# lovelyqian/Embodied-One-Shot-Video-Recognition

Measured on AMD Instinct MI355X. Metric: clips/sec/GPU (224², 8-seg) + 5-way-1-shot episode acc vs reference, higher is better.
Workload: dtype f32

## Files before the change

embodied-one-shot-video-recognition_amd/csrc/common.h:

```cpp
#pragma once

#include <hip/hip_runtime.h>

#include "eosv.h"

#include <cstdint>
#include <string>

namespace eosv {

#ifndef EOSV_BF16_RFIRST
#define EOSV_BF16_RFIRST 1
#endif

template <int N>
__device__ __forceinline__ void vm_wait() {
  static_assert(N >= 0 && N < 64, "vmcnt range");
  __builtin_amdgcn_s_waitcnt((N & 15) | ((N >> 4) << 14) | (7 << 4) | (15 << 8));
  asm volatile("" ::: "memory");
}

template <class V>
__device__ __forceinline__ void store_b128_guarded(V v, __amdgpu_buffer_rsrc_t r, int voff, int soff) {
#ifdef EOSV_STORE_GUARD_SB
  __builtin_amdgcn_sched_barrier(0);
  __builtin_amdgcn_raw_buffer_store_b128(v, r, voff, soff, 0);
  __builtin_amdgcn_sched_barrier(0);
  asm volatile("s_nop 0");
  __builtin_amdgcn_sched_barrier(0);
#elif defined(EOSV_STORE_GUARD_OFF)
  __builtin_amdgcn_raw_buffer_store_b128(v, r, voff, soff, 0);
#else
  __builtin_amdgcn_raw_buffer_store_b128(v, r, voff, soff, 0);
  asm volatile("s_nop 0" ::"v"(v));
#endif
}

namespace epi {
typedef float f32x2 __attribute__((ext_vector_type(2)));
typedef float f32x4 __attribute__((ext_vector_type(4)));
typedef __bf16 bf16x2 __attribute__((ext_vector_type(2)));
typedef short s16x2 __attribute__((ext_vector_type(2)));
__device__ __forceinline__ unsigned relu_bf2(f32x2 v) {
  const s16x2 h = __builtin_bit_cast(s16x2, __builtin_convertvector(v, bf16x2));
  return __builtin_bit_cast(unsigned, __builtin_elementwise_max(h, (s16x2){0, 0}));
}
__device__ __forceinline__ f32x2 bf2_f(unsigned u) {
  return (f32x2){__uint_as_float(u << 16), __uint_as_float(u & 0xffff0000u)};
}
__device__ __forceinline__ f32x2 pair_of(const f32x4& A, const f32x4& B, int k) {
  const f32x4 X = k >> 1 ? B : A;
  return k & 1 ? X.hi : X.lo;
}
}

void set_error(const std::string& msg);

#ifdef EOSV_PROFILING
int env_switch(const char* name, int dflt);
#define EOSV_ABL(a) ((a).abl)
#else
constexpr int env_switch(const char*, int dflt) { return dflt; }
#define EOSV_ABL(a) 0
#endif

#define EOSV_HIP_CHECK(expr)                                                               \
  do {                                                                                     \
    hipError_t _e = (expr);                                                                \
    if (_e != hipSuccess) {                                                                \
      ::eosv::set_error(std::string(#expr) + ": " + hipGetErrorString(_e));               \
      return EOSV_ERR_HIP;                                                                 \
    }                                                                                      \
  } while (0)

#define EOSV_LAUNCH_CHECK()                                                                \
  do {                                                                                     \
    hipError_t _e = hipGetLastError();                                                     \
    if (_e != hipSuccess) {                                                                \
      ::eosv::set_error(std::string("kernel launch: ") + hipGetErrorString(_e));          \
      return EOSV_ERR_HIP;                                                                 \
    }                                                                                      \
  } while (0)

struct LaunchInfo {
  long long blocks;
  long long slots;
};
int device_cu_count();
int kernel_occupancy(const void* kernel, int threads, size_t dyn_lds = 0);
inline int record_launch(LaunchInfo* info, long long blocks, long long per_cu) {
  info->blocks = blocks;
  info->slots = per_cu * device_cu_count();
  return EOSV_OK;
}

struct ConvArgs {
  const void* x;
  const void* w;
  const float* bias;
  const void* res;
  void* y;
  int N, H, W, Cin;
  int Ho, Wo, Cout;
  int KH, KW, KWp, stride, pad;
  int K;
  int relu;
  const void* zero;
  int abl;
  int xcd;
  int kcm;
  const void* x2;
  int H2, W2, Cin2, stride2, K1;
  int split;
  int xs, x2s;
  LaunchInfo* plan;
  float* kws;
  long long kws_bytes;
};
int conv_f32_ksplit_slices(const ConvArgs& a);

__host__ __device__ inline int split_chan(int c, int cin3) {
  const int c2 = 2 * (cin3 / 3);
  return c >= c2 ? c - c2 : c;
}
inline void conv_pixel_strides(ConvArgs& a) {
  if (!a.xs) a.xs = a.split ? 2 * (a.Cin / 3) : a.Cin;
  if (!a.x2s) a.x2s = a.split ? 2 * (a.Cin2 / 3) : a.Cin2;
}

__device__ __forceinline__ int xcd_tile(int b, int nb, int on) {
  if (!on) return b;
  const int q = nb >> 3, r = nb & 7, x = b & 7, i = b >> 3;
  return x * q + (x < r ? x : r) + i;
}

int launch_conv_f32(const ConvArgs& a, hipStream_t s);
int launch_conv_bf16(const ConvArgs& a, hipStream_t s);
bool conv_bf16_ts_ok(const ConvArgs& a);
int launch_conv_bf16_ts(const ConvArgs& a, hipStream_t s);
bool stem_pool_bf16_ok(int H, int W, bool direct);
int launch_stem_pool_bf16(const void* pack, int B, int H, int W, const void* w, const float* bias, void* y,
                          hipStream_t s, const float* frames = nullptr, LaunchInfo* info = nullptr);
bool stem_pool_x3_ok(int H, int W);
int launch_stem_pool_x3(const float* frames, int B, int H, int W, const void* w, const float* bias, void* y,
                        hipStream_t s, LaunchInfo* info = nullptr);
bool stem_pool_f32_ok(int H, int W);
bool stem_pool_f32_direct_ok(int H, int W);
int launch_stem_pool_f32(const void* pack, int B, int H, int W, const void* w, const float* bias, void* y,
                         hipStream_t s, bool split = false,
                         LaunchInfo* info = nullptr,
                         const float* frames = nullptr);
bool conv_rows_bf16_ok(const ConvArgs& a);
int launch_conv_rows_bf16(const ConvArgs& a, hipStream_t s);
bool conv_rowsr_bf16_ok(const ConvArgs& a);
int launch_conv_rowsr_bf16(const ConvArgs& a, hipStream_t s);
bool conv_s2rows_bf16_ok(const ConvArgs& a);
int launch_conv_s2rows_bf16(const ConvArgs& a, hipStream_t s);

struct Pair1x1Args {
  const void* x;
  const void* x2;
  const void* res;
  const void* w3;
  const float* b3;
  const void* w1;
  const float* b1;
  void* y;
  void* z;
  long long M;
  int c1, cds;
  LaunchInfo* plan;
  int cmid, cexp;
  int Ho, Wo, H2, W2;
  int abl;
  long long cap_elems;
};
bool pair1x1_bf16_ok(int cmid, int cexp, int c1, int cds, long long M);
int launch_pair1x1_bf16(const Pair1x1Args& a, hipStream_t s);
int launch_pair1x1r_bf16(const Pair1x1Args& a, hipStream_t s);
int pairw_tile(int cmid, int c1, int cds);
bool pairw_bf16_ok(int cmid, int cexp, int c1, int cds, long long M, long long cap_elems);
int launch_pairw_bf16(const Pair1x1Args& a, hipStream_t s);
struct BneckArgs {
  const void* x;
  const void* w1; const float* b1;
  const void* w2; const float* b2;
  const void* w3; const float* b3;
  const void* wn; const float* bn;
  void* y;
  void* z;
  int N, H, W, cin;
  LaunchInfo* plan;
  const void* res;
  int abl;
};
bool bneck_bf16_ok(int cin, int W, int H, int next);
int launch_bneck_bf16(const BneckArgs& a, hipStream_t s);
bool bneck_tail_bf16_ok(int W, int H);
int launch_bneck_tail_bf16(const BneckArgs& a, hipStream_t s);
bool bblock_bf16_ok(int W, int H);
int launch_bblock_bf16(const BneckArgs& a, hipStream_t s);
bool conv_rows_f32_ok(const ConvArgs& a);
int launch_conv_rows_f32(const ConvArgs& a, hipStream_t s);
bool conv_rows_x3_ok(const ConvArgs& a);
int launch_conv_rows_x3(const ConvArgs& a, hipStream_t s);

struct WinoDiv {
  unsigned m;
  int s;
};
inline WinoDiv wino_div(unsigned d) {
  int l = 0;
  while ((1ull << l) < d) ++l;
  return {(unsigned)((1ull << (31 + l)) / d + 1), 31 + l};
}
__host__ __device__ inline int wino_fdiv(int t, WinoDiv f) {
  return (int)(((unsigned long long)(unsigned)t * f.m) >> f.s);
}
struct WinoArgs {
  const float* x;
  const float* u;
  const float* bias;
  const float* res;
  float* y;
  int N, H, W, C;
  int relu;
  int xcd;
  int cbmajor;
  LaunchInfo* plan;
  int max_wg;
  WinoDiv dtt, dtw, dncb, dnmt;
};
inline size_t wino_u_index(int o, int i, int pos, int cin) {
  return ((((size_t)(o / 64) * (cin / 8) + i / 8) * 16 + pos) * 8 + i % 8) * 64 + o % 64;
}
bool conv_wino_f32_ok(int C);
int launch_conv_wino_f32(const WinoArgs& a, hipStream_t s);

__host__ __device__ inline int stem_row_pixels(int W, int pad) { return (W + 2 * pad + 1) & ~1; }
inline size_t stem_input_elems(int B, int H, int W, int pad) {
  return (size_t)B * (H + 2 * pad) * stem_row_pixels(W, pad) * 3 + 64;
}
int launch_pack_rgb_pad(const float* x, int B, int H, int W, int pad, void* y, int bf16, hipStream_t s);
int launch_maxpool3x3s2(const void* x, int B, int H, int W, int C, void* y, int Ho, int Wo,
                        int bf16, hipStream_t s);
int launch_avgpool(const void* x, int B, int HW, int C, float* y, int bf16, hipStream_t s);
int launch_act_to_f32(const void* x, long long n, int C, int mode, float* y, hipStream_t s);

}
```

embodied-one-shot-video-recognition_amd/csrc/eosv_api.hip:

```cpp
#include <hip/hip_bf16.h>

#include <cmath>
#include <cstdio>
#include <algorithm>
#include <cstring>
#include <string>
#include <unordered_map>
#include <vector>

#include "common.h"

#ifndef EOSV_F32_KCM_DEF
#define EOSV_F32_KCM_DEF 64
#endif

namespace eosv {

static thread_local std::string g_err;
void set_error(const std::string& msg) { g_err = msg; }

int device_cu_count() {
  static const int n = [] {
    int dev = 0, c = 0;
    if (hipGetDevice(&dev) != hipSuccess || hipDeviceGetAttribute(&c, hipDeviceAttributeMultiprocessorCount, dev) ||
// ... 330 lines not shown
  auto kidx = [&](int i, int y, int x) {
    return c.kcm ? ((size_t)(i / c.kcmc) * c.kh * c.kw + y * c.kw + x) * c.kcmc + i % c.kcmc
                 : ((size_t)y * c.kwp + x) * c.cinp + i;
  };
  for (int o = 0; o < c.cout; ++o)
    for (int i = 0; i < c.cin; ++i)
      for (int y = 0; y < c.kh; ++y)
        for (int x = 0; x < c.kw; ++x) {
          const float v = w[(((size_t)o * c.cin + i) * c.kh + y) * c.kw + x] * alpha[o];
          float* row = wf.data() + (size_t)o * c.K;
          if (!split) {
            row[kidx(i, y, x)] = v;
          } else {
            const float hi = bf_round_host(v);
            row[kidx(i, y, x)] = hi;
            row[kidx(c.cin + i, y, x)] = hi;
            row[kidx(2 * c.cin + i, y, x)] = bf_round_host(v - hi);
          }
        }
  return true;
}

static int upload_conv(eosv_handle* h, Conv& c, const Tensors& t, bool bf16, bool has_bn, Conv* ds = nullptr,
                       bool split = false) {
  std::vector<float> wf, beta, alpha;
  if (!fold_conv(c, t, bf16, has_bn, wf, beta, split, &alpha)) return EOSV_ERR_ARG;
  if (wino_eligible(h, c) && !ds) {
    std::vector<float> u((size_t)16 * c.cout * c.cin);
    const float* w = t.get(c.wname, (int64_t)c.cout * c.cin * 9);
    if (!w || eosv_wino_weights_f32(w, alpha.data(), c.cout, c.cin, u.data())) return EOSV_ERR_ARG;
    int urc;
    if ((urc = upload_bytes(h, (void**)&c.wu, &c.wubytes, u.data(), u.size() * 4))) return urc;
  }
  if (ds) {
    std::vector<float> wd, bd;
    if (!fold_conv(*ds, t, bf16, true, wd, bd, split)) return EOSV_ERR_ARG;
    if (ds->cout != c.cout || ds->kh != 1 || ds->K != c.kds) return set_error("fused downsample shape"), EOSV_ERR_ARG;
    const int Kt = c.K + c.kds;
    std::vector<float> wc((size_t)c.cout * Kt);
    for (int o = 0; o < c.cout; ++o) {
      std::copy(wf.begin() + (size_t)o * c.K, wf.begin() + (size_t)(o + 1) * c.K, wc.begin() + (size_t)o * Kt);
      std::copy(wd.begin() + (size_t)o * c.kds, wd.begin() + (size_t)(o + 1) * c.kds, wc.begin() + (size_t)o * Kt + c.K);
      beta[o] += bd[o];
    }
    wf.swap(wc);
  }
  int rc;
  if (bf16) {
    std::vector<unsigned short> wb(wf.size());
    for (size_t i = 0; i < wf.size(); ++i) wb[i] = f2bf_host(wf[i]);
    if ((rc = upload_bytes(h, &c.w, &c.wbytes, wb.data(), wb.size() * 2))) return rc;
  } else {
    if ((rc = upload_bytes(h, &c.w, &c.wbytes, wf.data(), wf.size() * 4))) return rc;
  }
  size_t bcap = c.b ? (size_t)c.cout * 4 : 0;
  return upload_bytes(h, (void**)&c.b, &bcap, beta.data(), (size_t)c.cout * 4);
}

static hipEvent_t prof_event(eosv_handle* h) {
  if (h->pool_used == h->pool.size()) {
    hipEvent_t e;
    if (hipEventCreate(&e) != hipSuccess) return nullptr;
    h->pool.push_back(e);
  }
  return h->pool[h->pool_used++];
}

static void add_plan_cost(eosv_handle* h, const LaunchInfo& li, double flops) {
  if (li.blocks <= 0 || li.slots <= 0) return;
  const double rounds = (double)((li.blocks + li.slots - 1) / li.slots);
  h->plan_cost += flops * rounds * (double)li.slots / (double)li.blocks;
}

#ifdef EOSV_PROFILING
__global__ __launch_bounds__(256) void lds_poison_kernel() {
  __shared__ unsigned lds[160 * 1024 / 4];
  volatile unsigned* p = lds;
  for (int i = threadIdx.x; i < 160 * 1024 / 4; i += 256) p[i] = 0xffffffffu;
}
static int poison_mode() { return env_switch("EOSV_POISON", 0); }
static void poison_lds(hipStream_t s) {
  if (poison_mode() & 4) (void)hipStreamSynchronize(s);
  if (poison_mode() & 2) hipLaunchKernelGGL(lds_poison_kernel, dim3(4 * device_cu_count()), dim3(256), 0, s);
  if (poison_mode() & 4) (void)hipStreamSynchronize(s);
}
static int poison_bufs(eosv_handle* h, hipStream_t s) {
  if (!(poison_mode() & 1)) return EOSV_OK;
  const size_t elt = act_bytes(h);
  for (void* p : h->buf) EOSV_HIP_CHECK(hipMemsetAsync(p, 0xff, (size_t)h->d.max_frames * h->act_elems * elt, s));
  for (void* p : h->sbuf)
    if (p) EOSV_HIP_CHECK(hipMemsetAsync(p, 0xff, (size_t)h->sub_frames * h->act_elems * elt, s));
  return EOSV_OK;
}
#else
static void poison_lds(hipStream_t) {}
static int poison_bufs(eosv_handle*, hipStream_t) { return EOSV_OK; }
#endif

static int run_conv(eosv_handle* h, const Conv& c, const void* x, int N, int H, int W, const void* res,
                    void* y, bool relu, bool bf16, hipStream_t s, const void* x2 = nullptr, int H2 = 0,
                    int W2 = 0, int stride2 = 1) {
  ConvArgs a{};
  a.x = x;
  a.w = c.w;
  a.bias = c.b;
  a.res = res;
  a.y = y;
  a.N = N;
  a.H = H;
  a.W = W;
  a.Cin = c.cinp;
  a.Ho = conv_out(H, c.kh, c.stride, c.pad);
  a.Wo = conv_out(W, c.kw, c.stride, c.pad);
  a.Cout = c.cout;
  a.KH = c.kh;
  a.KW = c.kw;
  a.KWp = c.kwp;
  a.stride = c.stride;
  a.pad = c.pad;
  a.K = c.K + (x2 ? c.kds : 0);
  a.relu = relu ? 1 : 0;
  if (x2) {
    a.x2 = x2;
    a.H2 = H2;
    a.W2 = W2;
    a.Cin2 = c.kds;
    a.stride2 = stride2;
    a.K1 = c.K;
  }
  a.zero = h->zero;
  static const int xcd = env_switch("EOSV_XCD", 1);
  a.xcd = xcd;
  a.kcm = c.kcm ? (bf16 ? 1 : c.kcmc) : 0;
  a.split = (bf16 && x3(h)) ? 1 : 0;
  a.xs = a.split ? 2 * c.cin : c.cinp;
  a.x2s = x2 ? (a.split ? 2 * (c.kds / 3) : c.kds) : 0;
  const double flops = 2.0 * N * a.Ho * a.Wo * c.cout *
                       ((double)c.kh * c.kw * c.cin + (x2 ? c.kds / (a.split ? 3 : 1) : 0));
  const bool wino = !bf16 && c.wu && !x2;
  WinoArgs wa{};
  if (wino) {
    wa.x = (const float*)x;
    wa.u = c.wu;
    wa.bias = c.b;
    wa.res = (const float*)res;
    wa.y = (float*)y;
    wa.N = N;
    wa.H = H;
    wa.W = W;
    wa.C = c.cin;
    wa.relu = a.relu;
    wa.xcd = xcd;
  }
  if (h->planning) {
    LaunchInfo li{};
    a.plan = wa.plan = &li;
    const int prc = wino ? launch_conv_wino_f32(wa, s) : bf16 ? launch_conv_bf16(a, s) : launch_conv_f32(a, s);
    if (prc == EOSV_OK) add_plan_cost(h, li, flops);
    return prc;
  }
  poison_lds(s);
  hipEvent_t e0 = nullptr, e1 = nullptr;
  if (h->prof) {
    e0 = prof_event(h);
    e1 = prof_event(h);
    if (!e0 || !e1) return set_error("profiling: hipEventCreate failed"), EOSV_ERR_HIP;
    EOSV_HIP_CHECK(hipEventRecord(e0, s));
  }
  const int rc = wino ? launch_conv_wino_f32(wa, s) : bf16 ? launch_conv_bf16(a, s) : launch_conv_f32(a, s);
  if (h->prof && rc == EOSV_OK) {
    EOSV_HIP_CHECK(hipEventRecord(e1, s));
    h->recs.push_back({c.id, e0, e1, flops});
  }
  return rc;
}

static bool pair_enabled() {
  static const bool v = env_switch("EOSV_PAIR", 1) != 0;
  return v;
}

static bool pairw_enabled() {
  static const bool v = env_switch("EOSV_PAIRW", 1) != 0;
  return v;
}

static long long act_buffer_elems(const eosv_handle* h) {
  const long long f = h->sub_frames > 0 ? std::min(h->sub_frames, h->d.max_frames) : h->d.max_frames;
  return f * (long long)h->act_elems;
}

static bool pair_ok(const eosv_handle* h, const Block& b, const Block* nb, long long M) {
  if (!pair_enabled() || !conv_bf(h) || x3(h) || !b.bottleneck || !nb || !nb->bottleneck) return false;
  const Conv &c3 = b.c3, &n1 = nb->c1;
  if (c3.kh != 1 || n1.kh != 1 || n1.stride != 1 || n1.cin != c3.cout) return false;
  if (c3.cin != 64) {
    const bool ds = b.has_ds && b.fuse_ds && b.ds.stride == 2 && b.c2.stride == 2;
    if (!pairw_enabled() || (b.has_ds && !ds)) return false;
    return pairw_bf16_ok(c3.cin, c3.cout, n1.cout, ds ? c3.kds : 0, M, act_buffer_elems(h));
  }
  if (b.c2.stride != 1 || (b.has_ds && !(b.fuse_ds && b.ds.stride == 1))) return false;
  return pair1x1_bf16_ok(c3.cin, c3.cout, n1.cout, b.has_ds ? c3.kds : 0, M);
}

static int run_pair(eosv_handle* h, const Block& b, const Block& nb, const void* x, const void* x2, const void* res,
                    void* y, void* z, long long M, hipStream_t s, int ho = 0, int wo = 0, int hin = 0, int win = 0) {
  Pair1x1Args p{};
  p.x = x;
  p.x2 = x2;
  p.res = res;
  p.w3 = b.c3.w;
  p.b3 = b.c3.b;
  p.w1 = nb.c1.w;
  p.b1 = nb.c1.b;
  p.y = y;
  p.z = z;
  p.M = M;
  p.c1 = nb.c1.cout;
  p.cds = x2 ? b.c3.kds : 0;
  p.cmid = b.c3.cin;
  p.cexp = b.c3.cout;
  p.Ho = ho;
  p.Wo = wo;
  p.H2 = hin;
  p.W2 = win;
  p.cap_elems = act_buffer_elems(h);
  const bool wide = p.cmid != 64;
  const double flops = 2.0 * M * ((double)b.c3.cout * (b.c3.cin + p.cds) + (double)nb.c1.cout * nb.c1.cin);
  if (h->planning) {
    LaunchInfo li{};
    p.plan = &li;
    const int prc = wide ? launch_pairw_bf16(p, s) : launch_pair1x1_bf16(p, s);
    if (prc == EOSV_OK) add_plan_cost(h, li, flops);
    return prc;
  }
  poison_lds(s);
  hipEvent_t e0 = nullptr, e1 = nullptr;
  if (h->prof) {
    e0 = prof_event(h);
    e1 = prof_event(h);
    if (!e0 || !e1) return set_error("profiling: hipEventCreate failed"), EOSV_ERR_HIP;
    EOSV_HIP_CHECK(hipEventRecord(e0, s));
  }
#ifdef EOSV_PROFILING
  static void* scr[3] = {nullptr, nullptr, nullptr};
  static size_t scr_b = 0;
  const bool selfcheck = (poison_mode() & 8) != 0;
  const size_t cap_b = (size_t)p.cap_elems * 2;
  if (selfcheck) {
    if (cap_b > scr_b) {
      for (auto& q : scr) {
        if (q) EOSV_HIP_CHECK(hipFree(q));
        q = nullptr;
        EOSV_HIP_CHECK(hipMalloc(&q, cap_b));
      }
      scr_b = cap_b;
    }
    if (res) EOSV_HIP_CHECK(hipMemcpyAsync(scr[0], res, cap_b, hipMemcpyDeviceToDevice, s));
  }
#endif
  const int rc = wide ? launch_pairw_bf16(p, s) : launch_pair1x1_bf16(p, s);
  if (h->prof && rc == EOSV_OK) {
    EOSV_HIP_CHECK(hipEventRecord(e1, s));
    h->recs.push_back({b.c3.id, e0, e1, flops});
  }
#ifdef EOSV_PROFILING
  if (selfcheck && rc == EOSV_OK) {
    Pair1x1Args q = p;
    if (res) q.res = scr[0];
    q.y = scr[1];
    q.z = scr[2];
    const int rc2 = wide ? launch_pairw_bf16(q, s) : launch_pair1x1_bf16(q, s);
    EOSV_HIP_CHECK(hipStreamSynchronize(s));
    const size_t ny = (size_t)M * p.cexp, nz = (size_t)M * p.c1;
    std::vector<unsigned short> a(ny), c(ny);
    long long dy = 0, dz = 0, fy = -1, fz = -1;
    EOSV_HIP_CHECK(hipMemcpy(a.data(), y, ny * 2, hipMemcpyDeviceToHost));
    EOSV_HIP_CHECK(hipMemcpy(c.data(), scr[1], ny * 2, hipMemcpyDeviceToHost));
    for (size_t i = 0; i < ny; ++i)
      if (a[i] != c[i] && dy++ == 0) fy = (long long)i;
    a.resize(nz);
    c.resize(nz);
    EOSV_HIP_CHECK(hipMemcpy(a.data(), z, nz * 2, hipMemcpyDeviceToHost));
    EOSV_HIP_CHECK(hipMemcpy(c.data(), scr[2], nz * 2, hipMemcpyDeviceToHost));
    for (size_t i = 0; i < nz; ++i)
      if (a[i] != c[i] && dz++ == 0) fz = (long long)i;
    fprintf(stderr, "pair selfcheck layer %d %s cmid %d c1 %d cds %d M %lld rc %d/%d: y differs %lld (first px %lld ch %lld), z %lld (first px %lld ch %lld)\n",
            b.c3.id, wide ? "pairw" : "pair1x1", p.cmid, p.c1, p.cds, M, rc, rc2, dy, fy < 0 ? -1 : fy / p.cexp,
            fy < 0 ? -1 : fy % p.cexp, dz, fz < 0 ? -1 : fz / p.c1, fz < 0 ? -1 : fz % p.c1);
  }
#endif
  return rc;
}

static bool bneck_enabled() {
  static const bool v = env_switch("EOSV_BNECK", 1) != 0;
  return v;
}

static bool bneck_eligible(const eosv_handle* h, const Block& b, int hh, int ww) {
  if (!bneck_enabled() || !conv_bf(h) || x3(h) || !b.bottleneck) return false;
  static const int mode = env_switch("EOSV_BNECK", 1);
  if ((mode == 2 && b.c1.cin != 256) || (mode == 3 && b.c1.cin != 64)) return false;
  const Conv &c1 = b.c1, &c2 = b.c2, &c3 = b.c3;
  if (c1.kh != 1 || c1.stride != 1 || c1.cout != 64 || c2.kh != 3 || c2.stride != 1 || c2.cin != 64 ||
      c2.cout != 64 || c2.kcm || c3.kh != 1 || c3.cin != 64 || c3.cout != 256)
    return false;
  if (b.has_ds ? !(b.fuse_ds && b.ds.stride == 1 && c1.cin == 64 && c3.kds == 64) : c1.cin != 256) return false;
  return bneck_bf16_ok(c1.cin, ww, hh, 0);
}

static bool last_in_stage(const eosv_handle* h, size_t bi) {
  for (size_t li = 0; li < 4; ++li)
    if (bi + 1 == h->stage_end[li]) return true;
  return false;
}

static int run_bneck(eosv_handle* h, const Block& b, const Block* nb, const void* x, void* y, void* z, int B, int hh,
                     int ww, hipStream_t s) {
  BneckArgs a{};
  a.x = x;
  a.w1 = b.c1.w;
// ... 557 lines not shown
```

embodied-one-shot-video-recognition_amd/eosv/_lib.py:

```python
from __future__ import annotations

import ctypes
import os

PKG_ROOT = os.path.dirname(os.path.dirname(os.path.abspath(__file__)))
LIB_PATH = os.environ.get("EOSV_LIBRARY") or os.path.join(PKG_ROOT, "libeosv.so")

def source_digest() -> str:
    import glob
    import hashlib

    h = hashlib.sha256()
    repo = os.path.dirname(PKG_ROOT)
    files = sorted(glob.glob(os.path.join(PKG_ROOT, "csrc", "*.hip"))) + \
        [os.path.join(PKG_ROOT, "csrc", "common.h"), os.path.join(repo, "include", "eosv.h"),
         os.path.join(PKG_ROOT, "csrc", "Makefile")]
    for f in files:
        h.update(os.path.basename(f).encode())
        with open(f, "rb") as fh:
            h.update(fh.read())
    return h.hexdigest()[:16]


def library_kind() -> str:
    name = os.path.basename(LIB_PATH)
    return "release" if name == "libeosv.so" else name


def library_digest() -> str:
    import hashlib

    if not os.path.exists(LIB_PATH):
        return ""
    with open(LIB_PATH, "rb") as fh:
        return hashlib.sha256(fh.read()).hexdigest()[:16]


EOSV_F32, EOSV_BF16, EOSV_F32X3 = 0, 1, 2
MATCH_PROTONET, MATCH_COSINE = 0, 1
MAX_COLS = 64

_STATUS = {-1: "EOSV_ERR_ARG", -2: "EOSV_ERR_HIP", -3: "EOSV_ERR_OOM",
           -4: "EOSV_ERR_UNSUPPORTED", -5: "EOSV_ERR_STATE"}

EXPORTS = ("eosv_create", "eosv_load_weights", "eosv_backbone_forward", "eosv_backbone_probe", "eosv_fc_forward",
           "eosv_clip_embed", "eosv_segment_mean", "eosv_match", "eosv_segment_match", "eosv_segment_match_episodes",
           "eosv_temporal_smooth", "eosv_normalize_frames", "eosv_crop_normalize_frames", "eosv_synth_frames", "eosv_plan_episodes", "eosv_profile_enable", "eosv_profile_read", "eosv_feature_dim", "eosv_device_bytes", "eosv_last_error",
           "eosv_destroy",
           "eosv_sgemm", "eosv_im2col", "eosv_col2im", "eosv_bn_workspace_bytes", "eosv_bn_train_forward",
           "eosv_bn_train_backward", "eosv_maxpool_forward", "eosv_maxpool_backward", "eosv_avgpool_forward",
           "eosv_broadcast_rows", "eosv_softmax_xent", "eosv_sum_rows", "eosv_add_bias", "eosv_sgd_momentum",
           "eosv_axpy", "eosv_nchw_to_nhwc", "eosv_conv2d_f32", "eosv_flip_weights",
           "eosv_sgemm_tn_splitk_workspace", "eosv_sgemm_tn_splitk", "eosv_conv_wgrad_f32_workspace",
           "eosv_conv_wgrad_f32", "eosv_conv2d_f32_workspace",
           "eosv_wino_weights_f32", "eosv_wino_weights_f32_device", "eosv_conv_wino_f32",
           "eosv_conv_wino_f32_grid",
           "eosv_conv_wgrad_wino_f32_workspace", "eosv_conv_wgrad_wino_f32",
           "eosv_stem_conv_f32", "eosv_stem_wgrad_f32_workspace", "eosv_stem_wgrad_f32",
           "eosv_sgemm_x3", "eosv_sgemm_x3_tn_splitk_workspace", "eosv_sgemm_x3_tn_splitk")


class EosvDesc(ctypes.Structure):
    _fields_ = [("arch", ctypes.c_int), ("dtype", ctypes.c_int), ("height", ctypes.c_int),
                ("width", ctypes.c_int), ("max_frames", ctypes.c_int), ("device", ctypes.c_int),
                ("num_classes", ctypes.c_int)]


class EosvError(RuntimeError):
    pass


_lib = None


def lib():
    global _lib
    if _lib is not None:
        return _lib
    if not os.path.exists(LIB_PATH):
        raise EosvError(f"{LIB_PATH} not built: run `make -C csrc` or __graft_entry__.build()")
    L = ctypes.CDLL(LIB_PATH, mode=os.RTLD_NOW | os.RTLD_LOCAL)
    vp, i32, i64, f32 = ctypes.c_void_p, ctypes.c_int, ctypes.c_int64, ctypes.c_float
    sig = {
        "eosv_create": (i32, [ctypes.POINTER(EosvDesc), ctypes.POINTER(vp)]),
        "eosv_load_weights": (i32, [vp, ctypes.POINTER(ctypes.c_char_p), ctypes.POINTER(vp),
                                    ctypes.POINTER(i64), i32]),
        "eosv_backbone_forward": (i32, [vp, vp, i32, vp, vp]),
        "eosv_backbone_probe": (i32, [vp, vp, i32, i32, vp, vp]),
        "eosv_fc_forward": (i32, [vp, vp, i32, vp, vp]),
        "eosv_clip_embed": (i32, [vp, vp, vp, i32, i32, i32, vp, vp]),
        "eosv_segment_mean": (i32, [vp, i32, i32, i32, vp, vp]),
        "eosv_match": (i32, [vp, vp, vp, vp, vp, i32, i32, i32, vp, vp, vp]),
        "eosv_segment_match": (i32, [vp, i32, vp, i32, i32, f32, f32, vp, vp, vp]),
        "eosv_segment_match_episodes": (i32, [vp, i32, i32, vp, i32, i32, f32, f32, vp, vp, vp]),
        "eosv_temporal_smooth": (i32, [vp, i32, i32, f32, f32, vp, vp]),
        "eosv_normalize_frames": (i32, [vp, i32, i32, i32, i32, vp, vp, vp, vp]),
        "eosv_crop_normalize_frames": (i32, [vp, i32, i32, i32, i32, i32, i32, i32, vp, vp, vp, vp]),
        "eosv_synth_frames": (i32, [vp, i32, i32, i32, vp, vp]),
        "eosv_plan_episodes": (i32, [vp, i32, i32, i32, ctypes.c_uint64, i32, vp, vp, vp]),
        "eosv_profile_enable": (i32, [vp, i32]),
        "eosv_profile_read": (i32, [vp, vp, vp, vp, i32]),
        "eosv_feature_dim": (i32, [vp]),
        "eosv_device_bytes": (i64, [vp]),
        "eosv_last_error": (ctypes.c_char_p, []),
        "eosv_destroy": (None, [vp]),
        "eosv_sgemm": (i32, [i32, i32, i32, i32, i32, f32, vp, i32, vp, i32, f32, vp, i32, vp]),
        "eosv_im2col": (i32, [vp, i32, i32, i32, i32, i32, i32, i32, i32, vp, vp]),
        "eosv_col2im": (i32, [vp, i32, i32, i32, i32, i32, i32, i32, i32, vp, vp]),
        "eosv_bn_workspace_bytes": (i64, [i32]),
        "eosv_bn_train_forward": (i32, [vp, i64, i32, vp, vp, f32, f32, vp, vp, vp, i32, vp, vp, vp, vp, vp, vp]),
        "eosv_bn_train_backward": (i32, [vp, vp, vp, i32, vp, i64, i32, vp, vp, vp, vp, vp, vp, vp, vp, vp]),
        "eosv_maxpool_forward": (i32, [vp, i32, i32, i32, i32, vp, vp, vp]),
        "eosv_maxpool_backward": (i32, [vp, vp, i32, i32, i32, i32, vp, vp]),
        "eosv_avgpool_forward": (i32, [vp, i32, i32, i32, vp, vp]),
        "eosv_broadcast_rows": (i32, [vp, i32, i32, i32, f32, vp, vp]),
        "eosv_softmax_xent": (i32, [vp, vp, i32, i32, vp, vp, vp]),
        "eosv_sum_rows": (i32, [vp, i32, i32, vp, i32, vp]),
        "eosv_add_bias": (i32, [vp, i32, i32, vp, vp]),
        "eosv_sgd_momentum": (i32, [vp, vp, vp, i64, f32, f32, i32, vp]),
        "eosv_axpy": (i32, [vp, vp, i64, f32, vp]),
        "eosv_nchw_to_nhwc": (i32, [vp, i32, i32, i32, i32, vp, vp]),
        "eosv_conv2d_f32": (i32, [vp, i32, i32, i32, i32, vp, i32, i32, i32, i32, i32, vp, vp, i32, vp, vp, i64,
                                  vp]),
        "eosv_conv2d_f32_workspace": (i64, [i32] * 9),
        "eosv_flip_weights": (i32, [vp, i32, i32, i32, i32, vp, vp]),
        "eosv_sgemm_tn_splitk_workspace": (i64, [i32, i32, i32]),
        "eosv_sgemm_tn_splitk": (i32, [i32, i32, i32, vp, i32, vp, i32, vp, i32, vp, i64, vp]),
        "eosv_conv_wgrad_f32_workspace": (i64, [i32] * 9),
        "eosv_conv_wgrad_f32": (i32, [vp, i32, i32, i32, i32, vp, i32, i32, i32, i32, i32, vp, vp, i64, vp]),
        "eosv_wino_weights_f32": (i32, [vp, vp, i32, i32, vp]),
        "eosv_wino_weights_f32_device": (i32, [vp, i32, i32, i32, vp, vp]),
        "eosv_conv_wino_f32": (i32, [vp, vp, vp, vp, i32, vp, i32, i32, i32, i32, vp]),
        "eosv_conv_wino_f32_grid": (i32, [vp, vp, vp, vp, i32, vp, i32, i32, i32, i32, vp, i32]),
        "eosv_conv_wgrad_wino_f32_workspace": (i64, [i32] * 4),
        "eosv_conv_wgrad_wino_f32": (i32, [vp, vp, i32, i32, i32, i32, vp, vp, i64, vp]),
        "eosv_stem_conv_f32": (i32, [vp, i32, i32, i32, vp, vp, vp]),
        "eosv_stem_wgrad_f32_workspace": (i64, [i32] * 3),
        "eosv_stem_wgrad_f32": (i32, [vp, vp, i32, i32, i32, vp, vp, i64, vp]),
        "eosv_sgemm_x3": (i32, [i32, i32, i32, i32, i32, f32, vp, i32, vp, i32, f32, vp, i32, vp, vp]),
        "eosv_sgemm_x3_tn_splitk_workspace": (i64, [i32, i32, i32]),
        "eosv_sgemm_x3_tn_splitk": (i32, [i32, i32, i32, vp, i32, vp, i32, vp, i32, vp, i64, vp]),
    }
    for name, (res, args) in sig.items():
        fn = getattr(L, name)
        fn.restype, fn.argtypes = res, args
    _lib = L
    return L


def check(rc: int, what: str):
    if rc != 0:
        msg = lib().eosv_last_error().decode(errors="replace")
        raise EosvError(f"{what} failed: {_STATUS.get(rc, rc)}: {msg}")


def ptr(t) -> int:
    return 0 if t is None else t.data_ptr()


def stream_ptr(stream=None) -> int:
    import torch

    s = stream if stream is not None else torch.cuda.current_stream()
    return s.cuda_stream
```

include/eosv.h:

```cpp
#ifndef EOSV_H
#define EOSV_H

#include <stdint.h>

#ifdef __cplusplus
extern "C" {
#endif

typedef struct ihipStream_t* eosv_stream_t;
typedef struct eosv_handle eosv_handle;

typedef enum {
  EOSV_OK = 0,
  EOSV_ERR_ARG = -1,
  EOSV_ERR_HIP = -2,
  EOSV_ERR_OOM = -3,
  EOSV_ERR_UNSUPPORTED = -4,
  EOSV_ERR_STATE = -5
} eosv_status;

typedef enum { EOSV_ARCH_R18 = 18, EOSV_ARCH_R50 = 50, EOSV_ARCH_R101 = 101 } eosv_arch;
typedef enum { EOSV_F32 = 0, EOSV_BF16 = 1, EOSV_F32X3 = 2 } eosv_dtype;
typedef enum { EOSV_MATCH_PROTONET = 0, EOSV_MATCH_COSINE = 1 } eosv_match_kind;

typedef struct {
  int arch;
  int dtype;
  int height;
  int width;
  int max_frames;
  int device;
  int num_classes;
} eosv_desc;

int eosv_create(const eosv_desc* desc, eosv_handle** out);

int eosv_load_weights(eosv_handle* h, const char* const* names, const void* const* host_ptrs,
                      const int64_t* numel, int n);

int eosv_backbone_forward(eosv_handle* h, const float* d_frames, int B, float* d_feat,
                          eosv_stream_t stream);

int eosv_fc_forward(eosv_handle* h, const float* d_feat, int B, float* d_logits,
                    eosv_stream_t stream);

int eosv_clip_embed(const float* d_feat, const int32_t* d_offsets, const int32_t* d_counts,
                    int n_clips, int D, int l2, float* d_emb, eosv_stream_t stream);

int eosv_segment_mean(const float* d_feat, int n_seg, int seg_len, int D, float* d_seg,
                      eosv_stream_t stream);

int eosv_match(const float* d_query, const float* d_support, const int32_t* d_sup_off,
               const int32_t* d_sup_slot, const int32_t* d_n_proto, int n_episodes, int D,
               int kind, int64_t* d_pred, float* d_score, eosv_stream_t stream);

int eosv_segment_match(const float* d_seg, int S, const float* d_gallery, int G, int D,
                       float lamda1, float lamda2, int64_t* d_ids, float* d_dist,
                       eosv_stream_t stream);

int eosv_segment_match_episodes(const float* d_seg, int n_episodes, int S, const float* d_gallery, int G,
                                int D, float lamda1, float lamda2, int64_t* d_ids, float* d_dist,
                                eosv_stream_t stream);

int eosv_temporal_smooth(const float* d_x, int rows, int cols, float lamda1, float lamda2,
                         float* d_y, eosv_stream_t stream);

int eosv_normalize_frames(const uint8_t* d_rgb, int n_frames, int H, int W, int crop, const float* mean,
                          const float* std, float* d_out, eosv_stream_t stream);

int eosv_crop_normalize_frames(const uint8_t* d_rgb, int n_frames, int H, int W, int crop, int top, int left,
                               int flip, const float* mean, const float* std, float* d_out, eosv_stream_t stream);

int eosv_synth_frames(const uint64_t* d_params, int n_frames, int H, int W, float* d_frames,
                      eosv_stream_t stream);

int eosv_profile_enable(eosv_handle* h, int enable);
int eosv_profile_read(eosv_handle* h, double* ms, double* flops, int64_t* launches, int max_layers);

int eosv_plan_episodes(const int32_t* class_sizes, int n_classes, int n_way, int k_shot, uint64_t seed,
                       int n_episodes, int32_t* classes, int32_t* query, int32_t* support);

int eosv_backbone_probe(eosv_handle* h, const float* d_frames, int B, int stage, float* d_out,
                        eosv_stream_t stream);


int eosv_sgemm(int trans_a, int trans_b, int m, int n, int k, float alpha, const float* d_a, int lda,
               const float* d_b, int ldb, float beta, float* d_c, int ldc, eosv_stream_t stream);
int64_t eosv_sgemm_tn_splitk_workspace(int m, int n, int k);
int eosv_sgemm_tn_splitk(int m, int n, int k, const float* d_a, int lda, const float* d_b, int ldb, float* d_c,
                         int ldc, float* d_work, int64_t work_bytes, eosv_stream_t stream);
int eosv_sgemm_x3(int trans_a, int trans_b, int m, int n, int k, float alpha, const float* d_a, int lda,
                  const float* d_b, int ldb, float beta, float* d_c, int ldc, const float* d_add,
                  eosv_stream_t stream);
int64_t eosv_sgemm_x3_tn_splitk_workspace(int m, int n, int k);
int eosv_sgemm_x3_tn_splitk(int m, int n, int k, const float* d_a, int lda, const float* d_b, int ldb, float* d_c,
                            int ldc, float* d_work, int64_t work_bytes, eosv_stream_t stream);
int64_t eosv_conv_wgrad_f32_workspace(int N, int H, int W, int Cin, int Cout, int KH, int KW, int stride, int pad);
int eosv_conv_wgrad_f32(const float* d_x, int N, int H, int W, int Cin, const float* d_dy, int Cout, int KH, int KW,
                        int stride, int pad, float* d_dw, float* d_work, int64_t work_bytes, eosv_stream_t stream);
int64_t eosv_conv_wgrad_wino_f32_workspace(int N, int H, int W, int C);
int eosv_conv_wgrad_wino_f32(const float* d_x, const float* d_dy, int N, int H, int W, int C, float* d_dw,
                             float* d_work, int64_t work_bytes, eosv_stream_t stream);
int eosv_stem_conv_f32(const float* d_frames, int N, int H, int W, const float* d_w, float* d_z,
                       eosv_stream_t stream);
int64_t eosv_stem_wgrad_f32_workspace(int N, int H, int W);
int eosv_stem_wgrad_f32(const float* d_frames, const float* d_dz, int N, int H, int W, float* d_dw, float* d_work,
                        int64_t work_bytes, eosv_stream_t stream);
int eosv_im2col(const float* d_x, int N, int H, int W, int C, int KH, int KW, int stride, int pad, float* d_col,
                eosv_stream_t stream);
int eosv_col2im(const float* d_col, int N, int H, int W, int C, int KH, int KW, int stride, int pad, float* d_x,
                eosv_stream_t stream);
int64_t eosv_bn_workspace_bytes(int C);
int eosv_bn_train_forward(const float* d_x, int64_t P, int C, const float* d_gamma, const float* d_beta, float eps,
                          float momentum, float* d_running_mean, float* d_running_var, const float* d_residual,
                          int relu, float* d_y, uint8_t* d_mask, float* d_save_mean, float* d_save_invstd,
                          void* d_work, eosv_stream_t stream);
int eosv_bn_train_backward(const float* d_dy, const float* d_y, const uint8_t* d_mask, int relu, const float* d_x,
                           int64_t P, int C, const float* d_gamma, const float* d_save_mean,
                           const float* d_save_invstd, float* d_dx, float* d_dgamma, float* d_dbeta, float* d_dres,
                           void* d_work, eosv_stream_t stream);
int eosv_maxpool_forward(const float* d_x, int N, int H, int W, int C, float* d_y, int32_t* d_idx,
                         eosv_stream_t stream);
int eosv_maxpool_backward(const float* d_dy, const int32_t* d_idx, int N, int H, int W, int C, float* d_dx,
                          eosv_stream_t stream);
int eosv_avgpool_forward(const float* d_x, int N, int HW, int C, float* d_y, eosv_stream_t stream);
int eosv_broadcast_rows(const float* d_dy, int N, int T, int C, float scale, float* d_dx, eosv_stream_t stream);
int eosv_softmax_xent(const float* d_logits, const int32_t* d_labels, int B, int C, float* d_row_loss,
                      float* d_dlogits, eosv_stream_t stream);
int eosv_sum_rows(const float* d_x, int rows, int C, float* d_y, int accumulate, eosv_stream_t stream);
int eosv_add_bias(float* d_y, int rows, int C, const float* d_bias, eosv_stream_t stream);
int eosv_sgd_momentum(float* d_p, const float* d_g, float* d_buf, int64_t n, float lr, float momentum, int first,
                      eosv_stream_t stream);
int eosv_conv2d_f32(const float* d_x, int N, int H, int W, int Cin, const float* d_w, int Cout, int KH, int KW,
                    int stride, int pad, const float* d_bias, const float* d_res, int relu, float* d_y, float* d_work,
                    int64_t work_bytes, eosv_stream_t stream);
int64_t eosv_conv2d_f32_workspace(int N, int H, int W, int Cin, int Cout, int KH, int KW, int stride, int pad);
int eosv_flip_weights(const float* d_w, int Cout, int KH, int KW, int Cin, float* d_wf, eosv_stream_t stream);
int eosv_axpy(float* d_y, const float* d_x, int64_t n, float alpha, eosv_stream_t stream);
int eosv_nchw_to_nhwc(const float* d_x, int N, int C, int H, int W, float* d_y, eosv_stream_t stream);

int eosv_wino_weights_f32(const float* w_ocihw, const float* alpha_or_null, int cout, int cin, float* u_out);
int eosv_wino_weights_f32_device(const float* d_w_ohwi, int cout, int cin, int flip, float* d_u,
                                 eosv_stream_t stream);
int eosv_conv_wino_f32(const float* d_x, const float* d_u, const float* d_bias, const float* d_res, int relu,
                       float* d_y, int N, int H, int W, int C, eosv_stream_t stream);
int eosv_conv_wino_f32_grid(const float* d_x, const float* d_u, const float* d_bias, const float* d_res, int relu,
                            float* d_y, int N, int H, int W, int C, eosv_stream_t stream, int max_workgroups);

int eosv_feature_dim(const eosv_handle* h);

int64_t eosv_device_bytes(const eosv_handle* h);

const char* eosv_last_error(void);
void eosv_destroy(eosv_handle* h);

#ifdef __cplusplus
}
#endif

#endif
```

Before: 3712.

## Add persistent MFMA f32 kernel for 1x1 downsample convolutions

Adds a dedicated persistent kernel for f32 1x1 convolutions without residual or relu, typically the ResNet downsample shortcut. It uses 32x32x2 f32 MFMA with double-buffered global-to-LDS loads, XOR-swizzled shared memory, and an epilogue that overlaps the previous tile's stores with the next tile's loads. The conv dispatch routes eligible layers (Cin up to 128, Cout a multiple of 128) to it instead of the generic f32 conv path. The grid is capped at one workgroup per CU, which may limit latency hiding, and stores are scalar per element.

After: 3714, median of 2. Within noise of the previous version (+0.0%).

```diff
diff --git a/embodied-one-shot-video-recognition_amd/csrc/common.h b/embodied-one-shot-video-recognition_amd/csrc/common.h
--- a/embodied-one-shot-video-recognition_amd/csrc/common.h
+++ b/embodied-one-shot-video-recognition_amd/csrc/common.h
@@ -150,6 +150,10 @@
                          hipStream_t s, bool split = false,
                          LaunchInfo* info = nullptr,
                          const float* frames = nullptr);
+bool conv1x1_f32_ok(const void* x, int N, int H, int W, int Cin, const void* w, int Cout, int stride, const void* bias,
+                    const void* y);
+int launch_conv1x1_f32(const float* x, int N, int H, int W, int Cin, const float* w, int Cout, int stride,
+                       const float* bias, float* y, hipStream_t s, LaunchInfo* plan = nullptr, int max_wg = 0);
 bool conv_rows_bf16_ok(const ConvArgs& a);
 int launch_conv_rows_bf16(const ConvArgs& a, hipStream_t s);
 bool conv_rowsr_bf16_ok(const ConvArgs& a);
diff --git a/embodied-one-shot-video-recognition_amd/csrc/conv1x1_f32.hip b/embodied-one-shot-video-recognition_amd/csrc/conv1x1_f32.hip
--- /dev/null
+++ b/embodied-one-shot-video-recognition_amd/csrc/conv1x1_f32.hip
@@ -0,0 +1,208 @@
+#include "common.h"
+
+#include <algorithm>
+
+namespace eosv {
+
+namespace {
+typedef float f32x4 __attribute__((ext_vector_type(4)));
+typedef float f32x16 __attribute__((ext_vector_type(16)));
+
+constexpr int C1_BM = 128, C1_BN = 128, C1_KC = 64;
+constexpr int C1_AS = C1_BM * C1_KC, C1_BS = C1_BN * C1_KC;
+constexpr int C1_SLOT = C1_AS + C1_BS;
+constexpr int C1_NT = 512;
+
+struct C1Args {
+  const float* x;
+  const float* w;
+  const float* bias;
+  float* y;
+  int H, W, Cin, Cout, stride;
+  int M;
+  int ncb, nkc;
+  int items;
+  WinoDiv dhw, dw, dcb;
+  int HoWo, Wo;
+};
+}
+
+__global__ __launch_bounds__(C1_NT) void conv1x1_f32_kernel(C1Args a) {
+  __shared__ __attribute__((aligned(16))) float smem[2 * C1_SLOT];
+  const int tid = threadIdx.x;
+  const int lane = tid & 63;
+  const int wid = __builtin_amdgcn_readfirstlane(tid >> 6);
+  const int wm = wid >> 1, wn = wid & 1;
+  const int h = lane >> 5, r = lane & 31;
+  const int G = gridDim.x;
+  const int wg = xcd_tile(blockIdx.x, G, 1);
+  const int nloc = (a.items - wg + G - 1) / G;
+  const int T = nloc * a.nkc;
+
+  const int lr = lane >> 4, pc = lane & 15;
+  int iit = wg, ikc = 0;
+  auto issue = [&](int slot, int half) {
+    const int pb = wino_fdiv(iit, a.dcb), cb = iit - pb * a.ncb;
+    float* As = smem + slot * C1_SLOT;
+    float* Bs = As + C1_AS;
+#pragma unroll
+    for (int j = 0; j < 4; ++j) {
+      const int row = 16 * wid + 4 * j + lr;
+      const int lc = pc ^ (row & 15);
+      const float* src;
+      if (half == 0) {
+        const int m = min(pb * C1_BM + row, a.M - 1);
+        const int n = wino_fdiv(m, a.dhw), rem = m - n * a.HoWo;
+        const int oh = wino_fdiv(rem, a.dw), ow = rem - oh * a.Wo;
+        src = a.x + ((long long)(n * a.H + oh * a.stride) * a.W + ow * a.stride) * a.Cin + ikc * C1_KC + lc * 4;
+      } else {
+        src = a.w + (long long)(cb * C1_BN + row) * a.Cin + ikc * C1_KC + lc * 4;
+      }
+      __builtin_amdgcn_global_load_lds((const void*)src,
+                                       (__attribute__((address_space(3))) void*)((half ? Bs : As) + (16 * wid + 4 * j) * C1_KC),
+                                       16, 0, 0);
+    }
+    if (half && ++ikc == a.nkc) ikc = 0, iit += G;
+  };
+
+  f32x16 acc[2], out[2];
+#pragma unroll
+  for (int j = 0; j < 2; ++j)
+#pragma unroll
+    for (int q = 0; q < 16; ++q) acc[j][q] = 0.f, out[j][q] = 0.f;
+  bool pend = false;
+  int opb = 0, ocb = 0;
+  float obias[2] = {0.f, 0.f};
+  auto store8 = [&](int q0) {
+#pragma unroll
+    for (int j = 0; j < 2; ++j) {
+      const int n = ocb * C1_BN + wn * 64 + j * 32 + r;
+#pragma unroll
+      for (int q = q0; q < q0 + 8; ++q) {
+        const int m = opb * C1_BM + wm * 32 + (q & 3) + 8 * (q >> 2) + 4 * h;
+        if (m < a.M) a.y[(long long)m * a.Cout + n] = out[j][q] + obias[j];
+      }
+    }
+  };
+
+  issue(0, 0);
+  issue(0, 1);
+  vm_wait<0>();
+  __builtin_amdgcn_s_barrier();
+  asm volatile("" ::: "memory");
+
+  const int arow = (wm * 32 + r) * C1_KC, brow = (wn * 64 + r) * C1_KC;
+  int it = wg, kc = 0;
+  for (int c = 0; c < T; ++c) {
+    const bool last = kc + 1 == a.nkc;
+    const bool more = c + 1 < T;
+    const int pb = wino_fdiv(it, a.dcb), cb = it - pb * a.ncb;
+    float bcol[2];
+#pragma unroll
+    for (int j = 0; j < 2; ++j) bcol[j] = (last && a.bias) ? a.bias[cb * C1_BN + wn * 64 + j * 32 + r] : 0.f;
+    const float* As = smem + (c & 1) * C1_SLOT;
+    const float* Bs = As + C1_AS;
+#pragma unroll
+    for (int t = 0; t < C1_KC / 16; ++t)
+#pragma unroll
+      for (int g = 0; g < 2; ++g) {
+        const int po = ((4 * t + 2 * h + g) ^ (r & 15)) * 4;
+        const f32x4 af = *(const f32x4*)(As + arow + po);
+        f32x4 bf[2];
+#pragma unroll
+        for (int j = 0; j < 2; ++j) bf[j] = *(const f32x4*)(Bs + brow + j * 32 * C1_KC + po);
+        const int idx = 2 * t + g;
+        if (idx < 2) {
+          if (more) issue((c + 1) & 1, idx);
+          if (pend) store8(8 * idx);
+        }
+#pragma unroll
+        for (int s = 0; s < 4; ++s)
+#pragma unroll
+          for (int j = 0; j < 2; ++j) acc[j] = __builtin_amdgcn_mfma_f32_32x32x2f32(af[s], bf[j][s], acc[j], 0, 0, 0);
+      }
+    asm volatile("s_waitcnt lgkmcnt(0)" ::: "memory");
+    vm_wait<0>();
+    __builtin_amdgcn_s_barrier();
+    asm volatile("" ::: "memory");
+    pend = last;
+    if (last) {
+#pragma unroll
+      for (int j = 0; j < 2; ++j) {
+        obias[j] = bcol[j];
+#pragma unroll
+        for (int q = 0; q < 16; ++q) out[j][q] = acc[j][q], acc[j][q] = 0.f;
+      }
+      opb = pb, ocb = cb;
+      kc = 0, it += G;
+    } else {
+      ++kc;
+    }
+  }
+  store8(0);
+  store8(8);
+  vm_wait<0>();
+}
+
+static bool conv1x1_f32_shape_ok(int Cin, int Cout, int stride) {
+  return Cin > 0 && Cin <= 256 && Cin % C1_KC == 0 && Cout > 0 && Cout % C1_BN == 0 && (stride == 1 || stride == 2);
+}
+
+bool conv1x1_f32_ok(const void* x, int N, int H, int W, int Cin, const void* w, int Cout, int stride, const void* bias,
+                    const void* y) {
+  if (!x || !w || !y || N <= 0 || H <= 0 || W <= 0 || !conv1x1_f32_shape_ok(Cin, Cout, stride)) return false;
+  if (((uintptr_t)x | (uintptr_t)w | (uintptr_t)y | (uintptr_t)bias) % 16) return false;
+  const long long Ho = (H - 1) / stride + 1, Wo = (W - 1) / stride + 1;
+  return (long long)N * H * W <= 0x7fffffffLL && (long long)N * Ho * Wo + C1_BM <= 0x7fffffffLL &&
+         ((long long)N * Ho * Wo + C1_BM - 1) / C1_BM * (Cout / C1_BN) <= 0x7fffffffLL;
+}
+
+int launch_conv1x1_f32(const float* x, int N, int H, int W, int Cin, const float* w, int Cout, int stride,
+                       const float* bias, float* y, hipStream_t s, LaunchInfo* plan, int max_wg) {
+  if (!x || !w || !y || N <= 0 || H <= 0 || W <= 0) return set_error("conv1x1_f32: bad argument"), EOSV_ERR_ARG;
+  if (!conv1x1_f32_ok(x, N, H, W, Cin, w, Cout, stride, bias, y))
+    return set_error("conv1x1_f32: needs Cin % 64 == 0, Cin <= 256, Cout % 128 == 0, stride 1 or 2, 16-byte aligned "
+                     "operands and fewer than 2^31 pixels"),
+           EOSV_ERR_UNSUPPORTED;
+  C1Args a{};
+  a.x = x;
+  a.w = w;
+  a.bias = bias;
+  a.y = y;
+  a.H = H;
+  a.W = W;
+  a.Cin = Cin;
+  a.Cout = Cout;
+  a.stride = stride;
+  const int Ho = (H - 1) / stride + 1, Wo = (W - 1) / stride + 1;
+  a.HoWo = Ho * Wo;
+  a.Wo = Wo;
+  a.M = N * Ho * Wo;
+  a.ncb = Cout / C1_BN;
+  a.nkc = Cin / C1_KC;
+  a.items = (int)(((long long)a.M + C1_BM - 1) / C1_BM * a.ncb);
+  a.dhw = wino_div((unsigned)a.HoWo);
+  a.dw = wino_div((unsigned)Wo);
+  a.dcb = wino_div((unsigned)a.ncb);
+  if (plan) return record_launch(plan, a.items, 1);
+  const int G = std::min(a.items, max_wg > 0 ? max_wg : device_cu_count());
+  hipLaunchKernelGGL(conv1x1_f32_kernel, dim3(G), dim3(C1_NT), 0, s, a);
+  EOSV_LAUNCH_CHECK();
+  return EOSV_OK;
+}
+
+}
+
+extern "C" int eosv_conv1x1_f32(const float* d_x, int N, int H, int W, int Cin, const float* d_w, int Cout, int stride,
+                                const float* d_bias, float* d_y, eosv_stream_t stream) {
+  return eosv::launch_conv1x1_f32(d_x, N, H, W, Cin, d_w, Cout, stride, d_bias, d_y, (hipStream_t)stream, nullptr, 0);
+}
+
+extern "C" int eosv_conv1x1_f32_grid(const float* d_x, int N, int H, int W, int Cin, const float* d_w, int Cout,
+                                     int stride, const float* d_bias, float* d_y, eosv_stream_t stream,
+                                     int max_workgroups) {
+  if (max_workgroups <= 0)
+    return eosv::set_error("eosv_conv1x1_f32_grid: max_workgroups must be positive"), EOSV_ERR_ARG;
+  return eosv::launch_conv1x1_f32(d_x, N, H, W, Cin, d_w, Cout, stride, d_bias, d_y, (hipStream_t)stream, nullptr,
+                                  max_workgroups);
+}
diff --git a/embodied-one-shot-video-recognition_amd/csrc/eosv_api.hip b/embodied-one-shot-video-recognition_amd/csrc/eosv_api.hip
--- a/embodied-one-shot-video-recognition_amd/csrc/eosv_api.hip
+++ b/embodied-one-shot-video-recognition_amd/csrc/eosv_api.hip
@@ -506,10 +506,21 @@
     wa.relu = a.relu;
     wa.xcd = xcd;
   }
+  static const bool ds1x1_on = env_switch("EOSV_F32_DS1X1", 1) != 0;
+  const bool ds1x1 = ds1x1_on && !bf16 && !wino && c.kh == 1 && c.kw == 1 && c.pad == 0 && !x2 && !res && !relu &&
+                     c.cinp == c.cin && c.cin <= 128 &&
+                     conv1x1_f32_ok(x, N, H, W, c.cin, c.w, c.cout, c.stride, c.b, y);
+  auto launch = [&](LaunchInfo* plan) {
+    if (wino) return launch_conv_wino_f32(wa, s);
+    if (ds1x1)
+      return launch_conv1x1_f32((const float*)x, N, H, W, c.cin, (const float*)c.w, c.cout, c.stride, c.b, (float*)y, s,
+                                plan);
+    return bf16 ? launch_conv_bf16(a, s) : launch_conv_f32(a, s);
+  };
   if (h->planning) {
     LaunchInfo li{};
     a.plan = wa.plan = &li;
-    const int prc = wino ? launch_conv_wino_f32(wa, s) : bf16 ? launch_conv_bf16(a, s) : launch_conv_f32(a, s);
+    const int prc = launch(&li);
     if (prc == EOSV_OK) add_plan_cost(h, li, flops);
     return prc;
   }
@@ -521,7 +532,7 @@
     if (!e0 || !e1) return set_error("profiling: hipEventCreate failed"), EOSV_ERR_HIP;
     EOSV_HIP_CHECK(hipEventRecord(e0, s));
   }
-  const int rc = wino ? launch_conv_wino_f32(wa, s) : bf16 ? launch_conv_bf16(a, s) : launch_conv_f32(a, s);
+  const int rc = launch(nullptr);
   if (h->prof && rc == EOSV_OK) {
     EOSV_HIP_CHECK(hipEventRecord(e1, s));
     h->recs.push_back({c.id, e0, e1, flops});
diff --git a/embodied-one-shot-video-recognition_amd/eosv/_lib.py b/embodied-one-shot-video-recognition_amd/eosv/_lib.py
--- a/embodied-one-shot-video-recognition_amd/eosv/_lib.py
+++ b/embodied-one-shot-video-recognition_amd/eosv/_lib.py
@@ -55,6 +55,7 @@
            "eosv_conv_wgrad_f32", "eosv_conv2d_f32_workspace",
            "eosv_wino_weights_f32", "eosv_wino_weights_f32_device", "eosv_conv_wino_f32",
            "eosv_conv_wino_f32_grid",
+           "eosv_conv1x1_f32", "eosv_conv1x1_f32_grid",
            "eosv_conv_wgrad_wino_f32_workspace", "eosv_conv_wgrad_wino_f32",
            "eosv_stem_conv_f32", "eosv_stem_wgrad_f32_workspace", "eosv_stem_wgrad_f32",
            "eosv_sgemm_x3", "eosv_sgemm_x3_tn_splitk_workspace", "eosv_sgemm_x3_tn_splitk")
@@ -132,6 +133,8 @@
         "eosv_wino_weights_f32_device": (i32, [vp, i32, i32, i32, vp, vp]),
         "eosv_conv_wino_f32": (i32, [vp, vp, vp, vp, i32, vp, i32, i32, i32, i32, vp]),
         "eosv_conv_wino_f32_grid": (i32, [vp, vp, vp, vp, i32, vp, i32, i32, i32, i32, vp, i32]),
+        "eosv_conv1x1_f32": (i32, [vp, i32, i32, i32, i32, vp, i32, i32, vp, vp, vp]),
+        "eosv_conv1x1_f32_grid": (i32, [vp, i32, i32, i32, i32, vp, i32, i32, vp, vp, vp, i32]),
         "eosv_conv_wgrad_wino_f32_workspace": (i64, [i32] * 4),
         "eosv_conv_wgrad_wino_f32": (i32, [vp, vp, i32, i32, i32, i32, vp, vp, i64, vp]),
         "eosv_stem_conv_f32": (i32, [vp, i32, i32, i32, vp, vp, vp]),
@@ -142,7 +145,11 @@
         "eosv_sgemm_x3_tn_splitk": (i32, [i32, i32, i32, vp, i32, vp, i32, vp, i32, vp, i64, vp]),
     }
     for name, (res, args) in sig.items():
-        fn = getattr(L, name)
+        fn = getattr(L, name, None)
+        if fn is None:
+            if os.environ.get("EOSV_LIBRARY"):
+                continue
+            raise EosvError(f"{LIB_PATH} lacks {name}: rebuild it")
         fn.restype, fn.argtypes = res, args
     _lib = L
     return L
diff --git a/include/eosv.h b/include/eosv.h
--- a/include/eosv.h
+++ b/include/eosv.h
@@ -147,6 +147,11 @@
 int eosv_conv_wino_f32_grid(const float* d_x, const float* d_u, const float* d_bias, const float* d_res, int relu,
                             float* d_y, int N, int H, int W, int C, eosv_stream_t stream, int max_workgroups);
 
+int eosv_conv1x1_f32(const float* d_x, int N, int H, int W, int Cin, const float* d_w, int Cout, int stride,
+                     const float* d_bias, float* d_y, eosv_stream_t stream);
+int eosv_conv1x1_f32_grid(const float* d_x, int N, int H, int W, int Cin, const float* d_w, int Cout, int stride,
+                          const float* d_bias, float* d_y, eosv_stream_t stream, int max_workgroups);
+
 int eosv_feature_dim(const eosv_handle* h);
 
 int64_t eosv_device_bytes(const eosv_handle* h);
```
